# Brockaaa/scenery-insitu

Measured on AMD Instinct MI355X. Metric: frames/sec @1920x1080 (8x512^3 volume), higher is better.
Workload: dtype f32

## Files before the change

scenery-insitu_amd/csrc/insitu_device.h:

```cpp
#pragma once
#include <hip/hip_runtime.h>
#include <stdint.h>

#pragma clang fp contract(off)

namespace insitu {

struct f4 {
    float x, y, z, w;
};

__device__ __forceinline__ float gmin(float x, float y) { return (y < x) ? y : x; }
__device__ __forceinline__ float gmax(float x, float y) { return (x < y) ? y : x; }
__device__ __forceinline__ float gmix(float x, float y, float a) { return __builtin_fmaf(y, a, x * (1.0f - a)); }

typedef float f2v __attribute__((ext_vector_type(2)));
__device__ __forceinline__ f2v pk_fma(f2v a, f2v b, f2v c) { return __builtin_elementwise_fma(a, b, c); }
__device__ __forceinline__ f2v lo2(const f4& v) { return f2v{v.x, v.y}; }
__device__ __forceinline__ f2v hi2(const f4& v) { return f2v{v.z, v.w}; }
__device__ __forceinline__ f4 join2(f2v a, f2v b) { return f4{a.x, a.y, b.x, b.y}; }

__device__ __forceinline__ f4 mat_vec(const float* m, f4 v) {
    const f2v r01 = pk_fma(f2v{m[12], m[13]}, f2v{v.w, v.w},
                           pk_fma(f2v{m[8], m[9]}, f2v{v.z, v.z},
// ... 7 lines not shown
    return __builtin_fmaf(m[12 + r], v.w, __builtin_fmaf(m[8 + r], v.z, __builtin_fmaf(m[4 + r], v.y, m[r] * v.x)));
}
__device__ __forceinline__ f4 v4mix(f4 a, f4 b, float t) {
    const float u = 1.0f - t;
    return join2(pk_fma(lo2(b), f2v{t, t}, lo2(a) * u), pk_fma(hi2(b), f2v{t, t}, hi2(a) * u));
}
__device__ __forceinline__ float len4(float x, float y, float z, float w) {
    return __builtin_sqrtf(__builtin_fmaf(w, w, __builtin_fmaf(z, z, __builtin_fmaf(y, y, x * x))));
}
__device__ __forceinline__ float len3(float x, float y, float z) {
    return __builtin_sqrtf(__builtin_fmaf(z, z, __builtin_fmaf(y, y, x * x)));
}
__device__ __forceinline__ f4 persp_div(f4 v) {
    float r = 1.0f / v.w;
    return f4{v.x * r, v.y * r, v.z * r, v.w * r};
}

__device__ __forceinline__ int xcd_block(int b, int nblocks, int C = 16) {
    const int span = 8 * C;
    if (b >= (nblocks / span) * span) return b;
    const int x = b & 7, i = b >> 3;
    return ((i / C) * 8 + x) * C + (i % C);
}

__host__ __device__ __forceinline__ float det_log2(float x) {
    const bool sub = x < 1.17549435e-38f;
    const float xs = sub ? x * 8388608.0f : x;
    const uint32_t u = __builtin_bit_cast(uint32_t, xs);
    int e = (int)((u >> 23) & 0xffu) - 127 + (sub ? -23 : 0);
    float m = __builtin_bit_cast(float, (u & 0x007fffffu) | 0x3f800000u);
    const bool big = m > 1.41421354f;
    m = big ? m * 0.5f : m;
    e += big ? 1 : 0;
    const float f = m - 1.0f;
#ifdef __HIP_DEVICE_COMPILE__
    const float dd = 2.0f + f;
    float y = __builtin_amdgcn_rcpf(dd);
    y = __builtin_fmaf(__builtin_fmaf(-dd, y, 1.0f), y, y);
    float s = f * y;
    s = __builtin_fmaf(__builtin_fmaf(-dd, s, f), y, s);
    s = __builtin_fmaf(__builtin_fmaf(-dd, s, f), y, s);
#else
    const float s = f / (2.0f + f);
#endif
    const float z = s * s;
    float p = __builtin_fmaf(z, 0.0909090936f, 0.111111112f);
    p = __builtin_fmaf(z, p, 0.142857149f);
    p = __builtin_fmaf(z, p, 0.200000003f);
    p = __builtin_fmaf(z, p, 0.333333343f);
    const float s2 = s + s;
    const float ln = __builtin_fmaf(s2 * z, p, s2);
    float r = __builtin_fmaf(ln, 1.44269502f, (float)e);
    r = (x == __builtin_inff()) ? __builtin_inff() : r;
    r = (x == 0.0f) ? -__builtin_inff() : r;
    r = (x >= 0.0f) ? r : __builtin_nanf("");
    return r;
}

__host__ __device__ __forceinline__ float det_exp2(float y) {
    const float n = __builtin_rintf(y);
    const float f = y - n;
    float p = 1.52527336e-05f;
    p = __builtin_fmaf(p, f, 1.54035297e-04f);
    p = __builtin_fmaf(p, f, 1.33335581e-03f);
    p = __builtin_fmaf(p, f, 9.61812911e-03f);
    p = __builtin_fmaf(p, f, 5.55041087e-02f);
    p = __builtin_fmaf(p, f, 2.40226507e-01f);
    p = __builtin_fmaf(p, f, 6.93147182e-01f);
    p = __builtin_fmaf(p, f, 1.0f);
    const float nc = __builtin_fminf(__builtin_fmaxf(n, -200.0f), 200.0f);
    const int ni = (int)nc;
    const int ea = ni > 127 ? 127 : (ni >= -126 ? ni : ni + 64);
    const float b = ni > 127 ? 2.0f : (ni >= -126 ? 1.0f : __builtin_bit_cast(float, (uint32_t)(127 - 64) << 23));
    float r = (p * __builtin_bit_cast(float, (uint32_t)(ea + 127) << 23)) * b;
    r = (y < -150.0f) ? 0.0f : r;
    r = (y >= 128.0f) ? __builtin_inff() : r;
    r = (y != y) ? y : r;
    return r;
}

__host__ __device__ __forceinline__ float det_pow(float x, float y) { return det_exp2(y * det_log2(x)); }
__host__ __device__ __forceinline__ float det_ln(float x) { return det_log2(x) * 0.693147182f; }

__host__ __device__ __forceinline__ float sq_threshold_search(float t) {
    if (!(t > 0.0f)) return 0.0f;
    float y = t * t;
    while (y > 0.0f && __builtin_sqrtf(y) >= t) y = __builtin_bit_cast(float, __builtin_bit_cast(uint32_t, y) - 1u);
    while (!(__builtin_sqrtf(y) >= t)) y = __builtin_bit_cast(float, __builtin_bit_cast(uint32_t, y) + 1u);
    return y;
}
__host__ __device__ __forceinline__ float sq_threshold(float t) {
    if (!(t >= 8.67361738e-19f && t <= 1.15292150e18f)) return sq_threshold_search(t);
    const uint32_t ut = __builtin_bit_cast(uint32_t, t);
    const float tm = __builtin_bit_cast(float, ut - 1u);
    const double mid = ((double)tm + (double)t) * 0.5;
    const double M = mid * mid;
    float y = (float)M;
    const bool even = (ut & 1u) == 0u;
    if ((double)y < M || ((double)y == M && !even)) y = __builtin_bit_cast(float, __builtin_bit_cast(uint32_t, y) + 1u);
    return y;
}
__device__ __forceinline__ float sumsq3(float x, float y, float z) {
    return __builtin_fmaf(z, z, __builtin_fmaf(y, y, x * x));
}

__device__ __forceinline__ float adjust_opacity(float a, float len) { return 1.0f - det_pow(1.0f - a, len); }

__device__ __forceinline__ uint32_t unorm8(float x) {
    float q = (x > 0.0f) ? ((x < 1.0f) ? x : 1.0f) : 0.0f;
    return (uint32_t)(int)__builtin_floorf(__builtin_fmaf(q, 255.0f, 0.5f));
}

__device__ __forceinline__ void texel_pair(float t, int n, int& i0, int& i1, float& frac) {
    float fl = __builtin_floorf(t);
    frac = t - fl;
    if (!(fl >= -1.0f)) fl = -1.0f;
    if (fl > (float)n) fl = (float)n;
    int i = (int)fl;
    i0 = i < 0 ? 0 : (i > n - 1 ? n - 1 : i);
    int j = i + 1;
    i1 = j < 0 ? 0 : (j > n - 1 ? n - 1 : j);
}

__device__ __forceinline__ uint32_t encode_depth_rgba8(float v) {
    float e0 = 1.0f * v, e1 = 255.0f * v, e2 = 65025.0f * v, e3 = 16581375.0f * v;
    e0 = e0 - __builtin_floorf(e0);
    e1 = e1 - __builtin_floorf(e1);
    e2 = e2 - __builtin_floorf(e2);
    e3 = e3 - __builtin_floorf(e3);
    const float c = 1.0f / 255.0f;
    float r0 = __builtin_fmaf(-e1, c, e0);
    float r1 = __builtin_fmaf(-e2, c, e1);
    float r2 = __builtin_fmaf(-e3, c, e2);
    float r3 = __builtin_fmaf(-e3, 0.0f, e3);
    return unorm8(r0) | (unorm8(r1) << 8) | (unorm8(r2) << 16) | (unorm8(r3) << 24);
}

__device__ __forceinline__ float decode_depth_rgba8(uint32_t p) {
    const float d0 = 1.0f, d1 = 1.0f / 255.0f, d2 = 1.0f / 65025.0f, d3 = 1.0f / 16581375.0f;
    float v0 = (float)(p & 0xffu) / 255.0f, v1 = (float)((p >> 8) & 0xffu) / 255.0f;
    float v2 = (float)((p >> 16) & 0xffu) / 255.0f, v3 = (float)(p >> 24) / 255.0f;
    return __builtin_fmaf(v3, d3, __builtin_fmaf(v2, d2, __builtin_fmaf(v1, d1, v0 * d0)));
}

}
```

scenery-insitu_amd/csrc/vdi_generate.hip:

```cpp
#include "insitu_sampling.h"
#include "insitu_filter.h"

#pragma clang fp contract(off)

namespace insitu {

__device__ __forceinline__ int find_z_interval_view(float z_view, float interval_size, int ncz) {
    float dist_from_front = __builtin_fabsf(z_view - (-1.0f * 0.1f));
    float q = __builtin_floorf(dist_from_front / interval_size);
    if (!(q < (float)ncz)) return ncz;
    return (int)q;
}

__host__ __device__ __forceinline__ size_t chunk_off(uint32_t c) { return (size_t)c * 64u; }

__host__ __device__ __forceinline__ size_t mslot_off(uint32_t c) { return (size_t)(c / 2u) * 128u + (c % 2u); }

struct RayOut {
    float4* color;
    float2* depth;
    uint32_t slot_stride;
};

__device__ __forceinline__ void octree_range(const VdiGenParams& P, float uvx, float uvy, float start, float end,
// ... 154 lines not shown
        if (close) {
            const int steps = s.steps_in;
            s.nterm++;
            s.open = false;
            s.endPt = ndc_of(s.tt_step + nw);
            s.steps_in = 0;
            s.steps_tt = 0;
            emit(s.startPt, s.endPt, DEFER ? s.curV : s.adj, steps);
        }
    }
    if (!s.open && !s.transparent) {
        s.open = true;
        s.startPt = ndc_of(stp);
        s.curV = f4{0.0f, 0.0f, 0.0f, 0.0f};
    }
    if (s.open) {
        s.curV = accumulate(s.curV, xv, wv);
        s.steps_in++;
        if (!s.transparent) {
            s.steps_tt = s.steps_in;
            s.tt_step = stp;
        }
    }
    if (last && s.open) {
        if (!DEFER) s.adj = exact_adjusted(s.curV, s.steps_tt, wfront, wback, nw);
        s.nterm++;
        s.open = false;
        s.endPt = ndc_of(s.tt_step + nw);
        s.steps_in = 0;
        emit(s.startPt, s.endPt, DEFER ? s.curV : s.adj, s.steps_tt);
    }
}

template <class Emit>
__device__ __forceinline__ void seg_sample_sel(SegState& s, const f4 xv, const float wv, const float stp, const bool on,
                                               const bool last, const Thr& th, const f4& wfront, const f4& wback,
                                               const float nw, Emit emit, const bool store) {
    const bool v = on && (xv.x > -0.5f || last);
    const bool tr = wv <= 0.0f;
    const bool o = v && s.open;
    const float a = approx_diff_sq(s.curV, s.steps_in, xv, wfront, wback, nw);
    const bool yes = a >= th.hi && a < 1.0e30f, no = a < th.lo;
    bool close = yes;
    const bool est = yes || no;
    float bnd = a;
    if (o && !est) {
        const f4 adj = exact_adjusted(s.curV, s.steps_in, wfront, wback, nw);
        bnd = exact_diff_sq(adj, xv);
        close = bnd >= th.sq;
        if (close) s.hi = __builtin_fminf(s.hi, bnd);
        else s.lo = __builtin_fmaxf(s.lo, bnd);
    }
    close = close && o;
    const bool eu = o && est;
    s.hi_a = __builtin_fminf(s.hi_a, (eu && close) ? a : __builtin_inff());
    s.lo_a = __builtin_fmaxf(s.lo_a, (eu && !close) ? a : -1.0f);
    if (close && store) emit(s.startPt, s.tt_step + nw, s.curV, s.steps_in);
    s.nterm += close ? 1 : 0;
    const bool open1 = s.open && !close;
    s.steps_in = close ? 0 : s.steps_in;
    s.steps_tt = close ? 0 : s.steps_tt;
    const bool opening = v && !open1 && !tr;
    s.startPt = opening ? stp : s.startPt;
    const f4 base{opening ? 0.0f : s.curV.x, opening ? 0.0f : s.curV.y, opening ? 0.0f : s.curV.z,
                  opening ? 0.0f : s.curV.w};
    const bool open2 = open1 || opening;
    const bool acc = v && open2;
    const f4 nv = accumulate(base, xv, wv);
    s.curV = f4{acc ? nv.x : base.x, acc ? nv.y : base.y, acc ? nv.z : base.z, acc ? nv.w : base.w};
    s.steps_in += acc ? 1 : 0;
    const bool tt = acc && !tr;
    s.steps_tt = tt ? s.steps_in : s.steps_tt;
    s.tt_step = tt ? stp : s.tt_step;
    const bool lc = v && last && open2;
    if (lc && store) emit(s.startPt, s.tt_step + nw, s.curV, s.steps_tt);
    s.nterm += lc ? 1 : 0;
    s.open = open2 && !lc;
    s.steps_in = lc ? 0 : s.steps_in;
}

struct CountStateL {
    f4 curV;
    int steps_in, nterm;
    bool open;
    float lo_a, hi_a;
    __device__ __forceinline__ void reset() {
        curV = f4{0.0f, 0.0f, 0.0f, 0.0f};
        steps_in = nterm = 0;
        open = false;
        lo_a = -1.0f;
        hi_a = __builtin_inff();
    }
};

template <bool FILTERED>
__device__ __forceinline__ void count_sample_l(CountStateL& s, float* bnd, const f4 xv, const float wv, const bool last,
                                               const Thr& th, const f4& wfront, const f4& wback, const float nw) {
    if (!(xv.x > -0.5f || last)) return;
    const bool transparent = wv <= 0.0f;
    if (s.open) {
        float b;
        bool est = false;
        if (close_decision<FILTERED>(s.curV, s.steps_in, xv, wfront, wback, nw, th, b, est)) {
            if (est) s.hi_a = __builtin_fminf(s.hi_a, b);
            else bnd[256] = __builtin_fminf(bnd[256], b);
            s.nterm++;
            s.open = false;
            s.steps_in = 0;
        } else {
            if (est) s.lo_a = __builtin_fmaxf(s.lo_a, b);
            else bnd[0] = __builtin_fmaxf(bnd[0], b);
        }
    }
    if (!s.open && !transparent) {
        s.open = true;
        s.curV = f4{0.0f, 0.0f, 0.0f, 0.0f};
    }
    if (s.open) {
        s.curV = accumulate(s.curV, xv, wv);
        s.steps_in++;
    }
    if (last && s.open) {
        s.nterm++;
        s.open = false;
    }
}

__device__ __forceinline__ float tree_threshold(float low, float high, float mid, int node) {
    const uint32_t m = (uint32_t)node + 1u;
    const int depth = 31 - __builtin_clz(m);
    for (int bit = depth - 1; bit >= 0; --bit) {
        if (((m >> bit) & 1u) == 0u) low = mid;
        else high = mid;
        mid = (low + high) / 2.0f;
    }
    return mid;
}

struct Search {
    float low, high, mid;
    int iter;
    bool found, written, first;
};

__device__ __forceinline__ void search_update(Search& q, int n, int S, int delta) {
    if (__builtin_fabsf(q.high - q.low) < 0.000001f) {
        q.found = true;
        q.mid = (n == 0) ? q.low : q.high;
        return;
    } else if (n > S) {
        q.low = q.mid;
    } else if (n < S - delta) {
        q.high = q.mid;
    } else {
        q.found = true;
        return;
    }
    if (q.first) {
        q.first = false;
        if (n < S) {
            q.found = true;
            return;
        }
    }
    q.mid = (q.low + q.high) / 2.0f;
}

__device__ __forceinline__ void search_step(Search& q, int n, int S, int delta, float lo, float hi, float4& iv,
                                            int& n_high) {
    if (!(__builtin_fabsf(q.high - q.low) < 0.000001f)) {
        if (n > S) {
            iv.x = lo;
            iv.y = hi;
        } else if (n < S - delta) {
            iv.z = lo;
            iv.w = hi;
            n_high = n;
        }
    }
    search_update(q, n, S, delta);
}

__device__ __forceinline__ void free_walk(Search& q, const float4 iv, int n_high, int S, int delta) {
    while (!q.found && q.iter < 63) {
        const float t = sq_threshold(q.mid);
        int n;
        if (t > iv.x && t <= iv.y) n = S + 1;
        else if (t > iv.z && t <= iv.w) n = n_high;
        else break;
        q.iter++;
        search_update(q, n, S, delta);
    }
}

__device__ __forceinline__ void store_slot(const RayOut& o, int i, float start, float end, const f4& c) {
    const uint32_t off = (uint32_t)i * o.slot_stride;
    o.color[off] = make_float4(c.x, c.y, c.z, c.w);
    o.depth[off] = make_float2(start, end);
}

__device__ __forceinline__ void finish_ray(const RayOut& o, int nseg, int S, uint8_t* passes, int iter) {
    (void)o;
    (void)nseg;
    (void)S;
    if (passes) *passes = (uint8_t)iter;
}

__device__ __forceinline__ float ndc_at(const VdiGenParams& P, const f4& wfront, const f4& wback, float t) {
    return persp_div(mat_vec(P.pv, v4mix(wfront, wback, t))).z;
}
__device__ __forceinline__ float ndc_at_rows(const float4* rows, const f4& wfront, const f4& wback, float t) {
    const f4 v = v4mix(wfront, wback, t);
    const float4 a = rows[0], b = rows[1];
    const float z = __builtin_fmaf(a.w, v.w, __builtin_fmaf(a.z, v.z, __builtin_fmaf(a.y, v.y, a.x * v.x)));
    const float w = __builtin_fmaf(b.w, v.w, __builtin_fmaf(b.z, v.z, __builtin_fmaf(b.y, v.y, b.x * v.x)));
    return z * (1.0f / w);
}

template <int DT, class SampleFn, class FlushFn>
__device__ __forceinline__ void march_pass(const VdiGenParams& P, const BrickDesc& brick, const float* s_tf,
                                           const float4* s_cm, const Ray& R, SampleFn sample_fn, FlushFn flush_fn) {
    const float nw = P.nw;
    float step = R.tnear;
    f4 wprev = v4mix(R.wfront, R.wback, step - nw);
    f4 wpos = v4mix(R.wfront, R.wback, step);
    bool in_cur = R.numSteps > 0 && step > R.localNear && step < R.localFar;
    float sc_cur;
    {
        VoxelFetch f;
        fetch_voxels<DT>(brick, wpos, f);
        sc_cur = voxel_coord(brick, f);
    }
    for (int i = 0; i < R.numSteps; ++i) {
        const bool last = (i == R.numSteps - 1);
        const float step_n = step + nw;
        const f4 wnext = v4mix(R.wfront, R.wback, step_n);
        const bool in_nxt = !last && step_n > R.localNear && step_n < R.localFar;
        VoxelFetch nxt;
        fetch_voxels<DT>(brick, wnext, nxt);
        if (in_cur) {
            const f4 x = classify_sample(sc_cur, s_tf, P.xfer.n_tf, s_cm, P.xfer.n_cm);
            float w = 0.0f;
            if (x.x > -0.5f || last)
                w = adjust_opacity(x.w, len4(wpos.x - wprev.x, wpos.y - wprev.y, wpos.z - wprev.z, wpos.w - wprev.w));
            if (!sample_fn(i, sc_cur, x, w, step, last)) break;
        }
        sc_cur = voxel_coord(brick, nxt);
        flush_fn();
        wprev = wpos;
        wpos = wnext;
        step = step_n;
        in_cur = in_nxt;
    }
}
template <int DT, class SampleFn>
__device__ __forceinline__ void march_pass(const VdiGenParams& P, const BrickDesc& brick, const float* s_tf,
                                           const float4* s_cm, const Ray& R, SampleFn sample_fn) {
    march_pass<DT>(P, brick, s_tf, s_cm, R, sample_fn, [] {});
}

template <int DT>
__device__ void vdi_march(const VdiGenParams& P, const BrickDesc& brick, uint32_t* octree, uint8_t* passes,
                          uint16_t* pending, const float* s_tf, const float4* s_cm, const Ray& R, const RayOut& o) {
    const float nw = P.nw;
    const int S = P.S;
    const int delta = (int)__builtin_floorf(0.15f * (float)S);
    int nseg = 0;
    Search q{0.0f, 1.732f, 0.0001f, 0, false, false, true};
    if (R.hit) {
        SegState st;
        auto ndc_of = [&](float t) { return ndc_at(P, R.wfront, R.wback, t); };
        while (!q.found || !q.written) {
            q.iter++;
            if (q.iter > 64) break;
            if (q.found) q.written = true;
            const Thr th{sq_threshold(q.mid), 0.0f, 0.0f};
            const bool write = q.found;
            st.reset();
            auto emit = [&](float s0, float e0, const f4& a, int) {
                if (write) {
                    if (nseg < S) store_slot(o, nseg, s0, e0, a);
                    octree_update(P, octree, R.uvx, R.uvy, s0, e0, R.cx, R.cy);
                    nseg++;
                }
            };
            march_pass<DT>(P, brick, s_tf, s_cm, R, [&](int, float, const f4& x, float w, float stp, bool last) {
                seg_sample(st, x, w, stp, ndc_of, last, th, R.wfront, R.wback, nw, emit);
                return write || st.nterm <= S;
            });
            if (!q.written) search_update(q, st.nterm, S, delta);
        }
    }
    *pending = (uint16_t)((nseg < S ? nseg : S) | kPendingCounted);
    finish_ray(o, nseg, S, passes, q.iter);
}

struct MultiRay {
    f4 wfront, wback;
    float uvx, uvy, tnear, tfar;
    float ln[kMaxBricks], lf[kMaxBricks];
    uint32_t vis;
    int cx, cy, numSteps;
};

__device__ __forceinline__ MultiRay multi_ray_setup(const VdiGenParams& P, int gx, int gy) {
    MultiRay r;
    Ray d;
    ray_dirs(P, gx, gy, d);
    r.wfront = d.wfront;
    r.wback = d.wback;
    r.uvx = d.uvx;
    r.uvy = d.uvy;
    r.cx = d.cx;
    r.cy = d.cy;
    r.tnear = 1.0f;
    r.tfar = 0.0f;
    r.vis = 0u;
#pragma unroll
    for (int v = 0; v < kMaxBricks; ++v) {
        r.ln[v] = 0.0f;
        r.lf[v] = 0.0f;
        if (v >= P.nvolumes) continue;
        float n, f;
        intersect_bbox(P.bricks[v], r.wfront, r.wback, n, f);
        f = gmin(P.tmax, f);
        if (n < f) {
            r.ln[v] = n;
            r.lf[v] = f;
            r.tnear = gmin(r.tnear, gmax(0.0f, n));
            r.tfar = gmax(r.tfar, f);
            r.vis |= 1u << v;
        }
    }
    r.numSteps = 0;
    if (r.tnear < r.tfar) {
        const float dsteps = __builtin_truncf((r.tfar - r.tnear) / P.nw);
        r.numSteps = (dsteps > 2.0e9f) ? 2000000000 : (int)dsteps;
    }
    return r;
}

template <int DT>
__device__ void merge_search_in_place(const VdiGenParams& P, const float* s_tf, const float4* s_cm, const MultiRay& R,
                                      const RayOut& o, int gx, int gy) {
    const float nw = P.nw;
    const int S = P.S;
    const int delta = (int)__builtin_floorf(0.15f * (float)S);
    int nseg = 0;
    Search q{0.0f, 1.732f, 0.0001f, 0, false, false, true};
    auto ndc_of = [&](float t) { return ndc_at(P, R.wfront, R.wback, t); };
    if (R.tnear < R.tfar) {
        SegState st;
        while (!q.found || !q.written) {
            q.iter++;
            if (q.iter > 64) break;
            if (q.found) q.written = true;
            const Thr th{sq_threshold(q.mid), 0.0f, 0.0f};
            const bool write = q.found;
            st.reset();
            auto emit = [&](float s0, float e0, const f4& a, int) {
                if (write) {
                    if (nseg < S) store_slot(o, nseg, s0, e0, a);
                    octree_update(P, P.octree, R.uvx, R.uvy, s0, e0, R.cx, R.cy);
                    nseg++;
                }
            };
            float step = R.tnear;
            f4 wprev = v4mix(R.wfront, R.wback, step - nw);
            bool decided = false;
            for (int i = 0; i < R.numSteps && !decided; ++i) {
                const bool last = (i == R.numSteps - 1);
                const f4 wpos = v4mix(R.wfront, R.wback, step);
                for (int v = 0; v < P.nvolumes; ++v) {
                    if (!((R.vis >> v) & 1u) || !(step > R.ln[v] && step < R.lf[v])) continue;
                    const BrickDesc& bk = P.bricks[v];
                    VoxelFetch f;
                    fetch_voxels<DT>(bk, wpos, f);
                    const float sc = voxel_coord(bk, f);
                    const f4 x = classify_sample(sc, s_tf, P.xfer.n_tf, s_cm, P.xfer.n_cm);
                    float w = 0.0f;
                    if (x.x > -0.5f || last)
                        w = adjust_opacity(x.w, len4(wpos.x - wprev.x, wpos.y - wprev.y, wpos.z - wprev.z, wpos.w - wprev.w));
                    seg_sample(st, x, w, step, ndc_of, last, th, R.wfront, R.wback, nw, emit);
                    if (!write && st.nterm > S) {
                        decided = true;
                        break;
                    }
                }
                wprev = wpos;
                step = step + nw;
            }
            if (!q.written) search_update(q, st.nterm, S, delta);
        }
    }
    P.seg_pending[(size_t)gy * (size_t)P.W + (size_t)gx] = (uint16_t)((nseg < S ? nseg : S) | kPendingCounted);
    finish_ray(o, nseg, S, P.passes ? P.passes + (size_t)gy * (size_t)P.W + (size_t)gx : nullptr, q.iter);
}

template <int DT, class SampleFn, class FlushFn>
__device__ __forceinline__ void march_multi(const VdiGenParams& P, const float* s_tf, const float4* s_cm,
                                            const MultiRay& R, SampleFn sample_fn, FlushFn flush_fn) {
    const float nw = P.nw;
    float step = R.tnear;
    f4 wprev = v4mix(R.wfront, R.wback, step - nw);
    uint32_t in = 0u, wm = 0u;
    float bnext = -__builtin_inff();
    for (int i = 0; i < R.numSteps; ++i) {
        const bool last = (i == R.numSteps - 1);
        const f4 wpos = v4mix(R.wfront, R.wback, step);
        if (__ballot(step >= bnext) != 0ull) {
            if (step >= bnext) {
                in = 0u;
                bnext = __builtin_inff();
#pragma unroll
                for (int v = 0; v < kMaxBricks; ++v) {
                    if (v >= P.nvolumes || !((R.vis >> v) & 1u)) continue;
                    if (step > R.ln[v] && step < R.lf[v]) in |= 1u << v;
                    if (step <= R.ln[v]) bnext = gmin(bnext, R.ln[v]);
                    if (step < R.lf[v]) bnext = gmin(bnext, R.lf[v]);
                }
            }
            wm = 0u;
#pragma unroll
            for (int v = 0; v < kMaxBricks; ++v)
                if (__ballot((in >> v) & 1u) != 0ull) wm |= 1u << v;
        }
        for (uint32_t m = wm; m != 0u; m &= m - 1u) {
            const int v = __builtin_ctz(m);
            if (!((in >> v) & 1u)) continue;
            const BrickDesc& bk = P.bricks[v];
            VoxelFetch f;
            fetch_voxels<DT>(bk, wpos, f);
            const float sc = voxel_coord(bk, f);
            const f4 x = classify_sample(sc, s_tf, P.xfer.n_tf, s_cm, P.xfer.n_cm);
            float w = 0.0f;
            if (x.x > -0.5f || last)
                w = adjust_opacity(x.w, len4(wpos.x - wprev.x, wpos.y - wprev.y, wpos.z - wprev.z, wpos.w - wprev.w));
            const bool go = sample_fn(i, sc, x, w, step, last);
            flush_fn();
            if (!go) return;
        }
        wprev = wpos;
        step = step + nw;
    }
}

struct PlainChunkStore {
    float4* first;
    __device__ __forceinline__ float4* at(uint32_t c) const { return first + 2 * chunk_off(c); }
    __device__ __forceinline__ void operator()(uint32_t c, const float4& cv, const float4& wv) const {
        float4* e = at(c);
        e[0] = cv;
        e[1] = wv;
    }
};
struct MergedChunkStore {
    float4* first;
    __device__ __forceinline__ float4* at(uint32_t c) const { return first + 4 * mslot_off(c); }
    __device__ __forceinline__ void pair(uint32_t c2, const float4& ca, const float4& wa, const float4& cb, const float4& wb,
                                         const uint4& s) const {
        float4* e = at(2 * c2);
        e[0] = ca;
        e[1] = wa;
        *reinterpret_cast<uint2*>(e + 2) = make_uint2(s.x, s.y);
        e[4] = cb;
        e[5] = wb;
        *reinterpret_cast<uint2*>(e + 6) = make_uint2(s.z, s.w);
    }
};

constexpr int kSpecLevels = 4;

template <int DT, bool FILTERED, bool MERGED, class March, class Store>
__device__ bool first_pass_impl(const VdiGenParams& P, const f4& wfront, const f4& wback, uint32_t cap_samples,
                                PendingRay& pr, float* p1, March march, Store store_fn) {
    const float nw = P.nw;
    const int S = P.S;
    const Thr th1 = uniform_thr(make_thr(sq_threshold(0.0001f), P.xfer.cmag));
    const int tid = threadIdx.x;
    float* const bl = p1 + tid;
    constexpr bool PAIRS = MERGED;
    float* const chk = p1 + 512 * (kSpecLevels + 1) + (PAIRS ? 20 : 8) * tid;
    CountStateL st;
    st.reset();
    const float root_mid = (0.0001f + 1.732f) / 2.0f;
    constexpr int K = kSpecLevels;
    static_assert(kSpecLevels >= 1);
    CountStateL cs[K];
    Thr tk[K];
#pragma unroll
    for (int l = 0, node = 0; l < K; ++l, node = 2 * node + 2) {
        cs[l].reset();
        tk[l] = uniform_thr(make_thr(sq_threshold(tree_threshold(0.0001f, 1.732f, root_mid, node)), P.xfer.cmag));
    }
#pragma unroll
    for (int l = 0; l <= K; ++l) {
        bl[512 * l] = 0.0f;
        bl[512 * l + 256] = __builtin_inff();
    }
    bool overflow = false;
    (void)cap_samples;
    int k = 0;
    float step_first = 0.0f;
    bool last_final = false;
    bool store_chunk = false;
    march([&](int i, float sc, const f4& x, float w, float stp, bool last) {
        const int j = k & 3;
        if constexpr (MERGED) {
            if ((uint32_t)k >= cap_samples) {
                overflow = true;
                return false;
            }
        } else {
            (void)i;
        }
        if constexpr (PAIRS) {
            const int pp = k & 7, h = pp >> 2;
            chk[8 * h + j] = sc;
            chk[8 * h + 4 + j] = w;
            reinterpret_cast<uint16_t*>(chk + 16)[pp] = (uint16_t)i;
            store_chunk = pp == 7 || last;
        } else {
            chk[j] = sc;
            chk[4 + j] = w;
            store_chunk = j == 3 || last;
        }
        if (k == 0) step_first = stp;
        k++;
        last_final = last;
        if (st.nterm <= S) count_sample_l<FILTERED>(st, bl, x, w, last, th1, wfront, wback, nw);
#pragma unroll
        for (int l = 0; l < K; ++l)
            if (cs[l].nterm <= S)
                count_sample_l<FILTERED>(cs[l], bl + 512 * (l + 1), x, w, last, tk[l], wfront, wback, nw);
        return true;
    }, [&] {
        if (store_chunk) {
            const float4 bc = *reinterpret_cast<const float4*>(chk), bw = *reinterpret_cast<const float4*>(chk + 4);
            if constexpr (PAIRS) {
                store_fn.pair((uint32_t)(k - 1) >> 3, bc, bw, *reinterpret_cast<const float4*>(chk + 8),
                              *reinterpret_cast<const float4*>(chk + 12), *reinterpret_cast<const uint4*>(chk + 16));
            } else {
                store_fn((uint32_t)(k - 1) >> 2, bc, bw);
            }
        }
        store_chunk = false;
    });
    if constexpr (MERGED) {
        if (overflow) return false;
    }
    if ((k & (PAIRS ? 7 : 3)) != 0 && !last_final) {
        const float4 bc = *reinterpret_cast<const float4*>(chk), bw = *reinterpret_cast<const float4*>(chk + 4);
        if constexpr (PAIRS) {
            store_fn.pair((uint32_t)k >> 3, bc, bw, *reinterpret_cast<const float4*>(chk + 8),
                          *reinterpret_cast<const float4*>(chk + 12), *reinterpret_cast<const uint4*>(chk + 16));
        } else {
            store_fn((uint32_t)k >> 2, bc, bw);
        }
    }
    if (st.nterm <= S) {
        pr.seg_low[0] = pr.seg_high[0] = __builtin_inff();
        pr.seg_low[1] = pr.seg_high[1] = -__builtin_inff();
        pr.n_high = 0u;
        pr.n = (uint32_t)k;
        pr.step_first = step_first;
        pr.last_final = last_final ? 1u : 0u;
        pr.low = 0.0f;
        pr.high = 1.732f;
        pr.mid = 0.0001f;
        pr.iter_found = 1u | 0x100u;
        return true;
    }
    const int delta = (int)__builtin_floorf(0.15f * (float)S);
    Search q{0.0001f, 1.732f, root_mid, 1, false, false, false};
    float lo[K + 1], hi[K + 1];
#pragma unroll
    for (int l = 0; l <= K; ++l) {
        lo[l] = bl[512 * l];
        hi[l] = bl[512 * l + 256];
        if constexpr (FILTERED) {
            const CountStateL& c = l == 0 ? st : cs[l > 0 ? l - 1 : 0];
            lo[l] = __builtin_fmaxf(lo[l], seg_lo_bound(c.lo_a, P.xfer.cmag));
            hi[l] = __builtin_fminf(hi[l], seg_hi_bound(c.hi_a, P.xfer.cmag));
        }
    }
    float4 iv{lo[0], hi[0], __builtin_inff(), -__builtin_inff()};
    int n_high = 0;
    bool on_spine = true;
#pragma unroll
    for (int l = 0; l < K; ++l) {
        if (!on_spine || q.found) break;
        q.iter++;
        on_spine = cs[l].nterm < S - delta && !(__builtin_fabsf(q.high - q.low) < 0.000001f);
        search_step(q, cs[l].nterm, S, delta, lo[l + 1], hi[l + 1], iv, n_high);
    }
    free_walk(q, iv, n_high, S, delta);
    pr.seg_low[0] = iv.x;
    pr.seg_low[1] = iv.y;
    pr.seg_high[0] = iv.z;
    pr.seg_high[1] = iv.w;
    pr.n_high = (uint32_t)n_high;
    pr.n = (uint32_t)k;
    pr.step_first = step_first;
    pr.last_final = last_final ? 1u : 0u;
    pr.low = q.low;
    pr.high = q.high;
    pr.mid = q.mid;
    pr.iter_found = (uint32_t)q.iter | (q.found ? 0x100u : 0u);
    return true;
}

template <int DT, bool FILTERED, class Store>
__device__ __forceinline__ bool vdi_first_pass(const VdiGenParams& P, const BrickDesc& brick, const float* s_tf,
                                               const float4* s_cm, const Ray& R, PendingRay& pr, float* p1, Store store_fn) {
    return first_pass_impl<DT, FILTERED, false>(P, R.wfront, R.wback, 0u, pr, p1, [&](auto sample_fn, auto flush_fn) {
        march_pass<DT>(P, brick, s_tf, s_cm, R, sample_fn, flush_fn);
    }, store_fn);
}

constexpr int kSampleXcdChunk = 4;
constexpr int kMergeMinBlocks = 3;
template <int DT, bool FILTERED>
__global__ __launch_bounds__(256, kMergeMinBlocks) void vdi_merge_kernel(const VdiGenParams P) {
    extern __shared__ __attribute__((aligned(16))) float4 smem[];
    float4* s_cm = smem;
    float* s_tf = reinterpret_cast<float*>(smem + lut_cm_slots(P.xfer.n_cm));
    stage_luts(P.xfer, s_cm, s_tf);
    const int wave = threadIdx.x >> 6, lane = threadIdx.x & 63;
    int tile = xcd_block((int)blockIdx.x, (int)gridDim.x) * 4 + wave;
    if (P.tile_ids) {
        const int ntiles = P.ytiles * P.nstrips * P.strip_tiles;
        const int j = xcd_block((int)blockIdx.x, (int)gridDim.x, kSampleXcdChunk) * 4 + wave;
        tile = j < ntiles ? (int)P.tile_ids[ntiles + j] : 4 * ntiles;
// ... 133 lines not shown
                const Ray R = ray_setup(P, P.bricks[b], d * P.strip_w + xl, gy);
                steps = R.hit ? R.numSteps : 0;
            }
        }
    }
#pragma unroll
    for (int o = 8; o > 0; o >>= 1) steps = max(steps, __shfl_xor(steps, o));
    if (s == 0 && tile < ntiles) {
        const uint32_t pos = (uint32_t)b * (uint32_t)ntiles + (uint32_t)tile;
        const uint32_t cls = (uint32_t)min(steps >> kTileClassShift, 255);
        P.tile_keys[pos] = (cls << 24) | (0xffffffu - pos);
        P.tile_ids[pos] = pos;
    }
}

template <int DT, bool FILTERED>
__device__ __forceinline__ void sample_tile(const VdiGenParams& P, const float* s_tf, const float4* s_cm, float* p1, int lane,
                                            int b, int tile) {
    const int yt = tile % P.ytiles;
    const int ct = tile / P.ytiles;
    const int d = ct / P.strip_tiles, xt = ct % P.strip_tiles;
    const int xx = lane & 7, yy = lane >> 3;
    const int xl = xt * 8 + xx, gy = yt * 8 + yy;
    const bool valid = d < P.nstrips && xl < P.strip_w && gy < P.H;
    const int gx = d * P.strip_w + xl;
    const BrickDesc& brick = P.bricks[b];
    Ray R{};
    if (valid) R = ray_setup(P, brick, gx, gy);

    float* cache = nullptr;
    uint32_t chunk = 0;
    unsigned long long base = 0;
    uint32_t total = 0;
    if (P.cache) {
        const uint32_t need = (valid && R.hit && R.numSteps < 65536) ? ((uint32_t)R.numSteps + 3u) >> 2 : 0u;
        uint32_t mx = need;
#pragma unroll
        for (int o = 32; o > 0; o >>= 1) mx = max(mx, (uint32_t)__shfl_xor((int)mx, o));
        total = mx * 64u;
        if (lane == 63 && total) base = atomicAdd(&P.ctr->cache_cursor, (unsigned long long)total);
        base = __shfl(base, 63);
        if (need && base + total <= (unsigned long long)P.cache_chunks) {
            chunk = (uint32_t)(base + (unsigned long long)lane);
            cache = P.cache + 8 * (size_t)chunk;
        }
    }
    {
        const unsigned long long mr = __ballot(valid && R.hit && R.numSteps > 0 && !cache);
        if (mr && lane == __builtin_ctzll(mr)) atomicAdd(&P.ctr->march_rays, (uint32_t)__popcll(mr));
    }
    bool pend = false;
    PendingRay pr{};
    if (valid) {
        const RayOut o = ray_out(P, gx, gy, b);
        uint32_t* oct = P.octree + (size_t)b * P.octree_stride;
        uint8_t* pas = P.passes ? P.passes + (size_t)b * P.passes_stride + (size_t)gy * (size_t)P.W + (size_t)gx
                                : nullptr;
        uint16_t* pnd = P.seg_pending + (size_t)b * P.passes_stride + (size_t)gy * (size_t)P.W + (size_t)gx;
        if (cache) {
            pend = vdi_first_pass<DT, FILTERED>(P, brick, s_tf, s_cm, R, pr, p1,
                                                PlainChunkStore{reinterpret_cast<float4*>(cache)});
            pr.pix = (uint32_t)gy * (uint32_t)P.W + (uint32_t)gx;
            pr.b = (uint32_t)b;
            pr.chunk = chunk;
        } else {
            vdi_march<DT>(P, brick, oct, pas, pnd, s_tf, s_cm, R, o);
        }
    }
    const bool lng = pend && pr.n >= P.long_samples;
    const unsigned long long ml = __ballot(lng), ms = __ballot(pend && !lng);
    uint32_t ql = 0, qs = 0;
    if (ml && lane == __builtin_ctzll(ml)) ql = atomicAdd(&P.ctr->queue_count, (uint32_t)__popcll(ml));
    if (ms && lane == __builtin_ctzll(ms)) qs = atomicAdd(&P.ctr->queue_short, (uint32_t)__popcll(ms));
    if (ml) ql = __shfl(ql, __builtin_ctzll(ml));
    if (ms) qs = __shfl(qs, __builtin_ctzll(ms));
    uint32_t slot = 0;
    if (pend) {
        const unsigned long long below = (1ull << lane) - 1ull;
        slot = lng ? ql + (uint32_t)__popcll(ml & below) : P.queue_cap - 1u - (qs + (uint32_t)__popcll(ms & below));
        P.queue[slot] = pr;
    }
}

constexpr int kSampleMinBlocks = 3;
template <int DT, bool FILTERED>
__global__ __launch_bounds__(256, kSampleMinBlocks) void vdi_sample_kernel(const VdiGenParams P) {
    extern __shared__ __attribute__((aligned(16))) float4 smem[];
    float4* s_cm = smem;
    float* s_tf = reinterpret_cast<float*>(smem + lut_cm_slots(P.xfer.n_cm));
    stage_luts(P.xfer, s_cm, s_tf);

    const int wave = threadIdx.x >> 6, lane = threadIdx.x & 63;
    const int lin = (int)(blockIdx.y * gridDim.x + blockIdx.x);
    const int logical = xcd_block(lin, (int)(gridDim.x * gridDim.y), kSampleXcdChunk);
    int b, tile;
    if (P.tile_ids) {
        const int ntiles = P.ytiles * P.nstrips * P.strip_tiles;
        const int j = logical * 4 + wave;
        const int total = P.B * ntiles;
        const uint32_t id = P.tile_ids[total + (j < total ? j : total - 1)];
        b = (int)(id / (uint32_t)ntiles);
        tile = j < total ? (int)(id - (uint32_t)b * (uint32_t)ntiles) : 4 * ntiles;
    } else {
        b = logical / (int)gridDim.x;
        tile = (logical - b * (int)gridDim.x) * 4 + wave;
    }
    b = __builtin_amdgcn_readfirstlane(b);
    tile = __builtin_amdgcn_readfirstlane(tile);
    sample_tile<DT, FILTERED>(P, s_tf, s_cm, reinterpret_cast<float*>(smem + lut_cm_slots(P.xfer.n_cm) + lut_tf_slots(P.xfer.n_tf)),
                              lane, b, tile);
}

constexpr int kSpecFrom = 8;
constexpr int kSpecFromGroup = 7;
constexpr int kSearchMinWaves = 3;
constexpr int kMaxSearchDepth = 6;
constexpr int kMaxRegroupDepth = 4;

constexpr int kP1LdsFloats = 512 * (kSpecLevels + 1) + 8 * 256;
__host__ __device__ __forceinline__ size_t sample_lds_bytes(int n_tf, int n_cm) {
    return lut_lds_bytes(n_tf, n_cm) + (size_t)kP1LdsFloats * 4;
}
__host__ __device__ __forceinline__ size_t merge_lds_bytes(int n_tf, int n_cm) {
    return lut_lds_bytes(n_tf, n_cm) + (size_t)(512 * (kSpecLevels + 1) + 20 * 256) * 4;
}

__host__ __device__ __forceinline__ size_t search_lds_bytes(int n_tf, int n_cm) {
    return lut_lds_bytes(n_tf, n_cm) + 4 * 256 * 16 + 256 * 4 + 2 * 16 + 256 * 4 + 256 * 8 + 256 * 8;
}

constexpr int kGroupBatch = 6;
constexpr float kDeepWindow = 3e-3f;
__device__ __forceinline__ Thr search_thr(float t_sq, float c, const Search& q) {
    Thr r = make_thr(t_sq, c);
    if (!q.found && q.high - q.low < kDeepWindow) {
        r.hi = __builtin_fmaxf(r.hi, make_thr(sq_threshold(q.high), c).hi);
        r.lo = __builtin_fminf(r.lo, make_thr(sq_threshold(q.low), c).lo);
    }
    return r;
}

template <bool FILTERED, bool MERGED>
__device__ __forceinline__ void search_loop(const VdiGenParams& P, float4* smem) {
    float4* s_cm = smem;
    float* s_tf = reinterpret_cast<float*>(smem + lut_cm_slots(P.xfer.n_cm));
    float4* s_c0 = smem + lut_cm_slots(P.xfer.n_cm) + lut_tf_slots(P.xfer.n_tf);
    float4* s_w0 = s_c0 + 256;
    float4* s_res = s_c0 + 512;
    float4* s_iv = s_c0 + 768;
    int* s_nh = reinterpret_cast<int*>(s_c0 + 1024);
    float4* s_pv = s_c0 + 1024 + 64;
    uint32_t* s_dbg_slot = reinterpret_cast<uint32_t*>(s_c0 + 1024 + 66);
    unsigned long long* s_dbg_t0 = reinterpret_cast<unsigned long long*>(s_c0 + 1024 + 66 + 64);
    uint2* s_s0 = reinterpret_cast<uint2*>(s_c0 + 1024 + 66 + 64 + 128);
    const int tid = threadIdx.x;
    const int lane = threadIdx.x & 63;
    GenCounters* const ctr = P.ctr;
    const uint32_t qlong = ctr->queue_count;
    const uint32_t qlen = qlong + ctr->queue_short;
    if (qlen == 0u) return;
    unsigned long long lanes = (unsigned long long)P.search_lanes;
    if (P.search_block_rays > 0) {
        uint32_t active = (qlen + (uint32_t)P.search_block_rays - 1u) / (uint32_t)P.search_block_rays;
        active = active < (uint32_t)P.search_min_blocks ? (uint32_t)P.search_min_blocks : active;
        if (blockIdx.x >= active) return;
        const unsigned long long al = (unsigned long long)active * 256ull;
        lanes = al < lanes ? al : lanes;
// ... 568 lines not shown
```

Before: 70.72.

## Add wave-uniform fast pow path and share paired count-state evaluation

Adds a fast det_pow path without special-case handling, chosen when the whole wave's inputs are normal and in range, and falls back to the full version otherwise. Paired threshold candidates (cs[0], cs[1]) now share one difference computation while their close decisions agree across the wave, and split back into separate states when they diverge. Replaces the open flag with a derived predicate and raises the sample kernel's minimum blocks per CU from 3 to 4. The changes add ballot overhead and more complex control flow, and the higher occupancy target may force register spills.

New measurement: 71.71 (median of 6 runs). +1.4%, better.

```diff
diff --git a/scenery-insitu_amd/csrc/insitu_device.h b/scenery-insitu_amd/csrc/insitu_device.h
--- a/scenery-insitu_amd/csrc/insitu_device.h
+++ b/scenery-insitu_amd/csrc/insitu_device.h
@@ -113,6 +113,53 @@
 __host__ __device__ __forceinline__ float det_pow(float x, float y) { return det_exp2(y * det_log2(x)); }
 __host__ __device__ __forceinline__ float det_ln(float x) { return det_log2(x) * 0.693147182f; }
 
+constexpr float kPowNormalLo = -125.0f, kPowNormalHi = 127.0f;
+__host__ __device__ __forceinline__ float det_log2_normal(float x) {
+    const uint32_t u = __builtin_bit_cast(uint32_t, x);
+    int e = (int)((u >> 23) & 0xffu) - 127;
+    float m = __builtin_bit_cast(float, (u & 0x007fffffu) | 0x3f800000u);
+    const bool big = m > 1.41421354f;
+    m = big ? m * 0.5f : m;
+    e += big ? 1 : 0;
+    const float f = m - 1.0f;
+#ifdef __HIP_DEVICE_COMPILE__
+    const float dd = 2.0f + f;
+    float y = __builtin_amdgcn_rcpf(dd);
+    y = __builtin_fmaf(__builtin_fmaf(-dd, y, 1.0f), y, y);
+    float s = f * y;
+    s = __builtin_fmaf(__builtin_fmaf(-dd, s, f), y, s);
+    s = __builtin_fmaf(__builtin_fmaf(-dd, s, f), y, s);
+#else
+    const float s = f / (2.0f + f);
+#endif
+    const float z = s * s;
+    float p = __builtin_fmaf(z, 0.0909090936f, 0.111111112f);
+    p = __builtin_fmaf(z, p, 0.142857149f);
+    p = __builtin_fmaf(z, p, 0.200000003f);
+    p = __builtin_fmaf(z, p, 0.333333343f);
+    const float s2 = s + s;
+    const float ln = __builtin_fmaf(s2 * z, p, s2);
+    return __builtin_fmaf(ln, 1.44269502f, (float)e);
+}
+__host__ __device__ __forceinline__ bool det_pow_normal_ok(float x, float y) {
+    const float t = y * det_log2_normal(x);
+    return x >= 1.17549435e-38f && x < __builtin_inff() && t >= kPowNormalLo && t <= kPowNormalHi;
+}
+__host__ __device__ __forceinline__ float det_pow_normal(float x, float y) {
+    const float t = y * det_log2_normal(x);
+    const float n = __builtin_rintf(t);
+    const float f = t - n;
+    float p = 1.52527336e-05f;
+    p = __builtin_fmaf(p, f, 1.54035297e-04f);
+    p = __builtin_fmaf(p, f, 1.33335581e-03f);
+    p = __builtin_fmaf(p, f, 9.61812911e-03f);
+    p = __builtin_fmaf(p, f, 5.55041087e-02f);
+    p = __builtin_fmaf(p, f, 2.40226507e-01f);
+    p = __builtin_fmaf(p, f, 6.93147182e-01f);
+    p = __builtin_fmaf(p, f, 1.0f);
+    return p * __builtin_bit_cast(float, (uint32_t)((int)n + 127) << 23);
+}
+
 __host__ __device__ __forceinline__ float sq_threshold_search(float t) {
     if (!(t > 0.0f)) return 0.0f;
     float y = t * t;
@@ -136,6 +183,11 @@
 }
 
 __device__ __forceinline__ float adjust_opacity(float a, float len) { return 1.0f - det_pow(1.0f - a, len); }
+__device__ __forceinline__ float adjust_opacity_wave(float a, float len) {
+    const float om = 1.0f - a;
+    if (__ballot(!det_pow_normal_ok(om, len)) == 0ull) return 1.0f - det_pow_normal(om, len);
+    return 1.0f - det_pow(om, len);
+}
 
 __device__ __forceinline__ uint32_t unorm8(float x) {
     float q = (x > 0.0f) ? ((x < 1.0f) ? x : 1.0f) : 0.0f;
diff --git a/scenery-insitu_amd/csrc/vdi_generate.hip b/scenery-insitu_amd/csrc/vdi_generate.hip
--- a/scenery-insitu_amd/csrc/vdi_generate.hip
+++ b/scenery-insitu_amd/csrc/vdi_generate.hip
@@ -260,12 +260,11 @@
 struct CountStateL {
     f4 curV;
     int steps_in, nterm;
-    bool open;
     float lo_a, hi_a;
+    __device__ __forceinline__ bool open() const { return steps_in > 0; }
     __device__ __forceinline__ void reset() {
         curV = f4{0.0f, 0.0f, 0.0f, 0.0f};
         steps_in = nterm = 0;
-        open = false;
         lo_a = -1.0f;
         hi_a = __builtin_inff();
     }
@@ -276,32 +275,98 @@
                                                const Thr& th, const f4& wfront, const f4& wback, const float nw) {
     if (!(xv.x > -0.5f || last)) return;
     const bool transparent = wv <= 0.0f;
-    if (s.open) {
+    if (s.open()) {
         float b;
         bool est = false;
         if (close_decision<FILTERED>(s.curV, s.steps_in, xv, wfront, wback, nw, th, b, est)) {
             if (est) s.hi_a = __builtin_fminf(s.hi_a, b);
             else bnd[256] = __builtin_fminf(bnd[256], b);
             s.nterm++;
-            s.open = false;
             s.steps_in = 0;
         } else {
             if (est) s.lo_a = __builtin_fmaxf(s.lo_a, b);
             else bnd[0] = __builtin_fmaxf(bnd[0], b);
         }
     }
-    if (!s.open && !transparent) {
-        s.open = true;
-        s.curV = f4{0.0f, 0.0f, 0.0f, 0.0f};
-    }
-    if (s.open) {
+    const bool opening = !s.open() && !transparent;
+    if (opening) s.curV = f4{0.0f, 0.0f, 0.0f, 0.0f};
+    if (s.open() || opening) {
         s.curV = accumulate(s.curV, xv, wv);
         s.steps_in++;
-    }
-    if (last && s.open) {
+        if (last) {
+            s.nterm++;
+            s.steps_in = 0;
+        }
+    }
+}
+
+__device__ __forceinline__ void count_apply_l(CountStateL& s, float& lo_a, float& hi_a, float* bnd, const bool v,
+                                              const bool o, const bool c, const bool est, const float b, const f4 xv,
+                                              const float wv, const bool last, const bool update) {
+    if (o) {
+        if (c) {
+            if (est) hi_a = __builtin_fminf(hi_a, b);
+            else bnd[256] = __builtin_fminf(bnd[256], b);
+        } else {
+            if (est) lo_a = __builtin_fmaxf(lo_a, b);
+            else bnd[0] = __builtin_fmaxf(bnd[0], b);
+        }
+    }
+    if (!update) return;
+    if (o && c) {
         s.nterm++;
-        s.open = false;
-    }
+        s.steps_in = 0;
+    }
+    if (v) {
+        const bool opening = !s.open() && !(wv <= 0.0f);
+        if (opening) s.curV = f4{0.0f, 0.0f, 0.0f, 0.0f};
+        if (s.open() || opening) {
+            s.curV = accumulate(s.curV, xv, wv);
+            s.steps_in++;
+            if (last) {
+                s.nterm++;
+                s.steps_in = 0;
+            }
+        }
+    }
+}
+template <bool FILTERED>
+__device__ __forceinline__ bool count_sample_pair(CountStateL& s0, CountStateL& s1, float* bnd0, float* bnd1, const int S,
+                                                  const f4 xv, const float wv, const bool last, const Thr& th0,
+                                                  const Thr& th1, const f4& wfront, const f4& wback, const float nw,
+                                                  const bool both) {
+    const bool v = s1.nterm <= S && (xv.x > -0.5f || last);
+    const bool o = v && s1.open();
+    bool c0 = false, c1 = false, e0 = false, e1 = false;
+    float a = 0.0f, ex = 0.0f;
+    if (o) {
+        if constexpr (FILTERED) {
+            a = approx_diff_sq(s1.curV, s1.steps_in, xv, wfront, wback, nw);
+            c1 = a >= th1.hi && a < 1.0e30f;
+            e1 = c1 || a < th1.lo;
+            if (both) {
+                c0 = a >= th0.hi && a < 1.0e30f;
+                e0 = c0 || a < th0.lo;
+            }
+        }
+        if (!e1 || (both && !e0)) {
+            ex = exact_diff_sq(exact_adjusted(s1.curV, s1.steps_in, wfront, wback, nw), xv);
+            if (!e1) c1 = ex >= th1.sq;
+            if (both && !e0) c0 = ex >= th0.sq;
+        }
+    }
+    bool split = false;
+    if (both) {
+        split = __ballot(c0 != c1) != 0ull;
+        if (split) {
+            s0.curV = s1.curV;
+            s0.steps_in = s1.steps_in;
+            s0.nterm = s1.nterm;
+        }
+        count_apply_l(s0, s0.lo_a, s0.hi_a, bnd0, v, o, c0, e0, e0 ? a : ex, xv, wv, last, split);
+    }
+    count_apply_l(s1, s1.lo_a, s1.hi_a, bnd1, v, o, c1, e1, e1 ? a : ex, xv, wv, last, true);
+    return both && !split;
 }
 
 __device__ __forceinline__ float tree_threshold(float low, float high, float mid, int node) {
@@ -420,7 +485,7 @@
             const f4 x = classify_sample(sc_cur, s_tf, P.xfer.n_tf, s_cm, P.xfer.n_cm);
             float w = 0.0f;
             if (x.x > -0.5f || last)
-                w = adjust_opacity(x.w, len4(wpos.x - wprev.x, wpos.y - wprev.y, wpos.z - wprev.z, wpos.w - wprev.w));
+                w = adjust_opacity_wave(x.w, len4(wpos.x - wprev.x, wpos.y - wprev.y, wpos.z - wprev.z, wpos.w - wprev.w));
             if (!sample_fn(i, sc_cur, x, w, step, last)) break;
         }
         sc_cur = voxel_coord(brick, nxt);
@@ -558,7 +623,7 @@
                     const f4 x = classify_sample(sc, s_tf, P.xfer.n_tf, s_cm, P.xfer.n_cm);
                     float w = 0.0f;
                     if (x.x > -0.5f || last)
-                        w = adjust_opacity(x.w, len4(wpos.x - wprev.x, wpos.y - wprev.y, wpos.z - wprev.z, wpos.w - wprev.w));
+                        w = adjust_opacity_wave(x.w, len4(wpos.x - wprev.x, wpos.y - wprev.y, wpos.z - wprev.z, wpos.w - wprev.w));
                     seg_sample(st, x, w, step, ndc_of, last, th, R.wfront, R.wback, nw, emit);
                     if (!write && st.nterm > S) {
                         decided = true;
@@ -613,7 +678,7 @@
             const f4 x = classify_sample(sc, s_tf, P.xfer.n_tf, s_cm, P.xfer.n_cm);
             float w = 0.0f;
             if (x.x > -0.5f || last)
-                w = adjust_opacity(x.w, len4(wpos.x - wprev.x, wpos.y - wprev.y, wpos.z - wprev.z, wpos.w - wprev.w));
+                w = adjust_opacity_wave(x.w, len4(wpos.x - wprev.x, wpos.y - wprev.y, wpos.z - wprev.z, wpos.w - wprev.w));
             const bool go = sample_fn(i, sc, x, w, step, last);
             flush_fn();
             if (!go) return;
@@ -682,6 +747,7 @@
     float step_first = 0.0f;
     bool last_final = false;
     bool store_chunk = false;
+    bool paired = K >= 2;
     march([&](int i, float sc, const f4& x, float w, float stp, bool last) {
         const int j = k & 3;
         if constexpr (MERGED) {
@@ -707,8 +773,22 @@
         k++;
         last_final = last;
         if (st.nterm <= S) count_sample_l<FILTERED>(st, bl, x, w, last, th1, wfront, wback, nw);
+        if constexpr (K >= 2) {
+            const bool both = __ballot(!paired) == 0ull;
+            if (!both) {
+                if (paired) {
+                    cs[0].curV = cs[1].curV;
+                    cs[0].steps_in = cs[1].steps_in;
+                    cs[0].nterm = cs[1].nterm;
+                    paired = false;
+                }
+                if (cs[0].nterm <= S) count_sample_l<FILTERED>(cs[0], bl + 512, x, w, last, tk[0], wfront, wback, nw);
+            }
+            paired = count_sample_pair<FILTERED>(cs[0], cs[1], bl + 512, bl + 1024, S, x, w, last, tk[0], tk[1], wfront,
+                                                 wback, nw, both);
+        }
 #pragma unroll
-        for (int l = 0; l < K; ++l)
+        for (int l = K >= 2 ? 2 : 0; l < K; ++l)
             if (cs[l].nterm <= S)
                 count_sample_l<FILTERED>(cs[l], bl + 512 * (l + 1), x, w, last, tk[l], wfront, wback, nw);
         return true;
@@ -727,6 +807,7 @@
     if constexpr (MERGED) {
         if (overflow) return false;
     }
+    if (paired) cs[0].nterm = cs[1].nterm;
     if ((k & (PAIRS ? 7 : 3)) != 0 && !last_final) {
         const float4 bc = *reinterpret_cast<const float4*>(chk), bw = *reinterpret_cast<const float4*>(chk + 4);
         if constexpr (PAIRS) {
@@ -1026,7 +1107,7 @@
     }
 }
 
-constexpr int kSampleMinBlocks = 3;
+constexpr int kSampleMinBlocks = 4;
 template <int DT, bool FILTERED>
 __global__ __launch_bounds__(256, kSampleMinBlocks) void vdi_sample_kernel(const VdiGenParams P) {
     extern __shared__ __attribute__((aligned(16))) float4 smem[];
```
